# cxm12/TGSR

Measured on AMD Instinct MI355X. Metric: SR images/sec (32->256, batch 16 per GPU, one step in flight), higher is better.
Workload: dtype f32

## Files before the change

### include/tgsr_hip.h

```cpp
#ifndef TGSR_HIP_H
#define TGSR_HIP_H

#include <stdint.h>

#ifdef __cplusplus
extern "C" {
#endif

#define TGSR_OK 0
#define TGSR_EINVAL (-1)
#define TGSR_EUNSUPPORTED (-2)
#define TGSR_ELAUNCH (-3)

#define TGSR_EPI_AFFINE 0
#define TGSR_EPI_AFFINE_GLU 1

#define TGSR_ACT_NONE 0
#define TGSR_ACT_TANH_AXPY 1
#define TGSR_ACT_IDENT_AXPY 2

#define TGSR_ABI_VERSION 2
int tgsr_abi_version(void);
const char* tgsr_last_error(void);

int64_t tgsr_packed_weight_elems(int Cout, int Cin, int K);
int tgsr_pack_conv_weight(const float* w, float* wpack, int Cout, int Cin, int K, void* stream);
int tgsr_pack_conv_weight_dgrad(const float* w, float* wpack, int Cout, int Cin, int K, void* stream);

int tgsr_bn_fold(const float* weight, const float* bias, const float* running_mean, const float* running_var,
                 float eps, float* scale, float* shift, int C, void* stream);

int tgsr_conv3x3_fwd(const float* x, int64_t x_bstride, int B, int Cin, int H, int W, const float* wpack, int Cout,
                     const float* scale, const float* shift, const float* residual, int64_t res_bstride, float* out,
                     int64_t out_bstride, int epilogue, int upsample, void* stream);
int tgsr_conv3x3_fwd_plan(int B, int H, int W, int Cout, int epilogue, int upsample, int* nob, int* rows_per_wave, int* groups);

int64_t tgsr_packed_upconv_weight_elems(int Cout, int Cin);
int tgsr_pack_upconv_weight(const float* w, float* wpack, int Cout, int Cin, void* stream);
int tgsr_upconv3x3_glu_fwd(const float* x, int64_t x_bstride, int B, int Cin, int H, int W, const float* wpack, int Cout,
                           const float* scale, const float* shift, float* out, int64_t out_bstride, void* stream);

int64_t tgsr_packed_upwino_weight_elems(int Cout, int Cin);
int tgsr_pack_upwino_weight(const float* w, float* upack, int Cout, int Cin, int glu, void* stream);
int tgsr_upwino_glu_fwd(const float* x, int64_t x_bstride, int B, int Cin, int H, int W, const float* upack, int Cout,
                        const float* scale, const float* shift, float* out, int64_t out_bstride, void* stream);
int tgsr_upwino_fwd(const float* x, int64_t x_bstride, int B, int Cin, int H, int W, const float* upack, int Cout,
                    const float* scale, const float* shift, float* out, int64_t out_bstride, void* stream);

int64_t tgsr_packed_upwino4_weight_elems(int Cout, int Cin);
int tgsr_pack_upwino4_weight(const float* w, float* upack, int Cout, int Cin, int glu, void* stream);
int tgsr_upwino4_fwd(const float* x, int64_t x_bstride, int B, int Cin, int H, int W, const float* upack, int Cout,
                     const float* scale, const float* shift, float* out, int64_t out_bstride, int glu, void* stream);

int64_t tgsr_packed_wino_weight_elems(int Cout, int Cin);
int tgsr_pack_wino_weight(const float* w, float* upack, int Cout, int Cin, int glu, void* stream);
int tgsr_pack_wino_weight_dgrad(const float* w, float* upack, int Cout, int Cin, void* stream);
int tgsr_wino_conv3x3_fwd(const float* x, int64_t x_bstride, int B, int Cin, int H, int W, const float* upack, int Cout,
                          const float* scale, const float* shift, const float* residual, int64_t res_bstride,
                          float* out, int64_t out_bstride, int epilogue, void* stream);

int64_t tgsr_packed_wino4_weight_elems(int Cout, int Cin);
int tgsr_pack_wino4_weight(const float* w, float* upack, int Cout, int Cin, int glu, void* stream);
int tgsr_pack_wino4_weight_dgrad(const float* w, float* upack, int Cout, int Cin, void* stream);
int tgsr_wino4_conv3x3_fwd(const float* x, int64_t x_bstride, int B, int Cin, int H, int W, const float* upack, int Cout,
                           const float* scale, const float* shift, const float* residual, int64_t res_bstride,
                           float* out, int64_t out_bstride, int epilogue, void* stream);

int tgsr_pack_wino4_wide_weight(const float* w, float* upack, int Cout, int Cin, int glu, void* stream);
int tgsr_pack_wino4_wide_weight_dgrad(const float* w, float* upack, int Cout, int Cin, void* stream);
int tgsr_wino4_wide_stats_nslots(int B, int H, int W, int Cout);
int tgsr_wino4_wide_conv3x3_stats_fwd(const float* x, int64_t x_bstride, int B, int Cin, int H, int W, const float* upack,
                                      int Cout, float* out, int64_t out_bstride, float* stat_partial, void* stream);
int tgsr_wino4_wide_conv3x3_fwd(const float* x, int64_t x_bstride, int B, int Cin, int H, int W, const float* upack, int Cout,
                                const float* scale, const float* shift, const float* residual, int64_t res_bstride,
                                float* out, int64_t out_bstride, int epilogue, void* stream);

#define TGSR_CONV_FORM_DIRECT 0
#define TGSR_CONV_FORM_UPCONV 1
#define TGSR_CONV_FORM_UPWINO 2
#define TGSR_CONV_FORM_UPWINO4 3
#define TGSR_CONV_FORM_WINO 4
#define TGSR_CONV_FORM_WINO4 5
#define TGSR_CONV_FORM_WINO4W 6
#define TGSR_CONV_FORMS 7
#define TGSR_CONV_PLAN_FIELDS 15
int tgsr_conv3x3_form_plan(int form, const float* x, int64_t x_bstride, int B, int Cin, int H, int W, const float* pack, int Cout,
                           const float* scale, const float* shift, const float* residual, int64_t res_bstride, const float* out,
                           int64_t out_bstride, int epilogue, int upsample, int stats, int* plan);

int tgsr_conv_to3_set_pipe(int on);

int tgsr_conv_to3_fwd(const float* x, int64_t x_bstride, int B, int Cin, int H, int W, const float* w, int K,
                      int act, const float* addend, float alpha, float* out, void* stream);
#define TGSR_TO3_FORM_MFMA 0
#define TGSR_TO3_FORM_PIPE 1
#define TGSR_TO3_FORM_VEC4 2
#define TGSR_TO3_FORM_SCALAR 3
int tgsr_conv_to3_plan(const float* x, int64_t x_bstride, int B, int Cin, int H, int W, int K, const float* addend,
                       const float* out, int* form, int* tile_rows);

int tgsr_conv_to3_finish_fwd(const float* x, int64_t x_bstride, int B, int Cin, int H, int W, const float* w, int K, float* out,
                             int n, float* const* fine, const float* const* t, const float* const* s, const int64_t* numel,
                             float alpha, void* stream);

int tgsr_word_attention_fwd(const float* h, int64_t h_bstride, const float* words, const float* w_ctx,
                            const uint8_t* mask, int mask_mode, int B, int idf, int cdf, int T, int Q, float* src_ws,
                            float* c_code, int64_t c_bstride, float* attn, void* stream);

int tgsr_word_project_fwd(const float* words, const float* const* w_ctx, int nsets, int B, int idf, int cdf, int T,
                          float* src_out, void* stream);

int tgsr_bilstm_fwd(const int64_t* captions, int width, const int32_t* cap_lens, int B, int Tmax, const float* emb,
                    int ntoken, int ninput, const float* w_ih, const float* w_hh, const float* b_ih,
                    const float* b_hh, int H, float* gates_ws, float* words_emb, float* sent_emb, void* stream);

int tgsr_lstm_gate_table(const float* emb, int ntoken, int ninput, const float* w_ih, const float* b_ih,
                         const float* b_hh, int H, float* table, void* stream);
int tgsr_bilstm_table_fwd(const int64_t* captions, int width, const int32_t* cap_lens, int B, int Tmax,
                          const float* table, int ntoken, const float* w_hh, int H, float* words_emb, float* sent_emb,
                          void* stream);

#define TGSR_LSTM_RECURRENT2_128 1
#define TGSR_LSTM_RECURRENT_128 2
#define TGSR_LSTM_RECURRENT_64 3
#define TGSR_LSTM_RECURRENT_32 4
#define TGSR_LSTM_RECURRENT_GENERIC 5
int tgsr_lstm_recurrent_plan(int H, int Tmax);

// ... 327 lines not shown
```

### tgsr_amd/_lib.py

```python
import ctypes
import os
import subprocess

_HERE = os.path.dirname(os.path.abspath(__file__))
LIB_PATH = os.environ.get("TGSR_LIB_PATH") or os.path.join(_HERE, "lib", "libtgsr_hip.so")
ABI_VERSION = 2

OK, EINVAL, EUNSUPPORTED, ELAUNCH = 0, -1, -2, -3
EPI_AFFINE, EPI_AFFINE_GLU = 0, 1
ACT_NONE, ACT_TANH_AXPY, ACT_IDENT_AXPY = 0, 1, 2
TO3_FORM_MFMA, TO3_FORM_PIPE, TO3_FORM_VEC4, TO3_FORM_SCALAR = 0, 1, 2, 3
DT_BF16, DT_F16 = 1, 2
WGRAD_DIRECT, WGRAD_WINO, WGRAD_UPWINO = 0, 1, 2
WGRAD_FAMILIES = ("conv3x3_wgrad_kernel<%d,%d,%s>", "wino_wgrad_kernel<%d,%d>", "wino_wgrad_dma_kernel<%d>", "upwino_wgrad_kernel<%d>")
WGRAD_PLAN_FIELDS, WGRAD_PLAN_WS = 10, 9
TO3_BWD_PLAN_FIELDS, TO3_BWD_PLAN_WS = 4, 3
CONV_FORMS = ("direct", "upconv", "upwino", "upwino4", "wino", "wino4", "wino4w")
CONV_FAMILIES = ("conv3x3_mfma_kernel<%d,%s,%s,%d,4>", "upconv_glu_mfma_kernel", "upwino_kernel<%s>", "upwino4_kernel<%s>",
                 "wino_conv3x3_kernel<%s,%d,%s>", "wino4_conv3x3_kernel<%s,%s>", "wino4w_conv3x3_kernel<%s,%d,%s>")
CONV_PLAN_FIELDS = 15
(CONV_PLAN_FAMILY, CONV_PLAN_T, CONV_PLAN_GRID_X, CONV_PLAN_GRID_Y, CONV_PLAN_BLOCK, CONV_PLAN_TILES_X, CONV_PLAN_TILES_Y,
 CONV_PLAN_TILE_H, CONV_PLAN_TILE_W, CONV_PLAN_STAGES, CONV_PLAN_GROUPS, CONV_PLAN_NSLOTS) = (0, 1, 5, 6, 7, 8, 9, 10, 11, 12, 13, 14)

LSTM_RECURRENT = {1: "lstm_recurrent2_kernel<128,24,4>", 2: "lstm_recurrent_kernel<128>", 3: "lstm_recurrent_kernel<64>",
                  4: "lstm_recurrent_kernel<32>", 5: "lstm_recurrent_generic_kernel"}
LSTM_RECURRENT_GENERIC = 5

_vp, _i, _i64, _f, _d = ctypes.c_void_p, ctypes.c_int, ctypes.c_int64, ctypes.c_float, ctypes.c_double

SIGNATURES = {
    "tgsr_abi_version": (_i, []),
    "tgsr_last_error": (ctypes.c_char_p, []),
    "tgsr_packed_weight_elems": (_i64, [_i, _i, _i]),
    "tgsr_pack_conv_weight": (_i, [_vp, _vp, _i, _i, _i, _vp]),
    "tgsr_pack_conv_weight_dgrad": (_i, [_vp, _vp, _i, _i, _i, _vp]),
    "tgsr_bn_fold": (_i, [_vp, _vp, _vp, _vp, _f, _vp, _vp, _i, _vp]),
    "tgsr_conv3x3_fwd": (_i, [_vp, _i64, _i, _i, _i, _i, _vp, _i, _vp, _vp, _vp, _i64, _vp, _i64, _i, _i, _vp]),
    "tgsr_conv3x3_fwd_plan": (_i, [_i, _i, _i, _i, _i, _i, _vp, _vp, _vp]),
    "tgsr_packed_upconv_weight_elems": (_i64, [_i, _i]),
    "tgsr_pack_upconv_weight": (_i, [_vp, _vp, _i, _i, _vp]),
    "tgsr_upconv3x3_glu_fwd": (_i, [_vp, _i64, _i, _i, _i, _i, _vp, _i, _vp, _vp, _vp, _i64, _vp]),
    "tgsr_packed_upwino_weight_elems": (_i64, [_i, _i]),
    "tgsr_pack_upwino_weight": (_i, [_vp, _vp, _i, _i, _i, _vp]),
    "tgsr_upwino_glu_fwd": (_i, [_vp, _i64, _i, _i, _i, _i, _vp, _i, _vp, _vp, _vp, _i64, _vp]),
    "tgsr_upwino_fwd": (_i, [_vp, _i64, _i, _i, _i, _i, _vp, _i, _vp, _vp, _vp, _i64, _vp]),
    "tgsr_packed_upwino4_weight_elems": (_i64, [_i, _i]),
    "tgsr_pack_upwino4_weight": (_i, [_vp, _vp, _i, _i, _i, _vp]),
    "tgsr_upwino4_fwd": (_i, [_vp, _i64, _i, _i, _i, _i, _vp, _i, _vp, _vp, _vp, _i64, _i, _vp]),
    "tgsr_packed_wino_weight_elems": (_i64, [_i, _i]),
    "tgsr_pack_wino_weight": (_i, [_vp, _vp, _i, _i, _i, _vp]),
    "tgsr_pack_wino_weight_dgrad": (_i, [_vp, _vp, _i, _i, _vp]),
    "tgsr_wino_conv3x3_fwd": (_i, [_vp, _i64, _i, _i, _i, _i, _vp, _i, _vp, _vp, _vp, _i64, _vp, _i64, _i, _vp]),
    "tgsr_packed_wino4_weight_elems": (_i64, [_i, _i]),
    "tgsr_pack_wino4_weight": (_i, [_vp, _vp, _i, _i, _i, _vp]),
    "tgsr_pack_wino4_weight_dgrad": (_i, [_vp, _vp, _i, _i, _vp]),
    "tgsr_pack_wino4_wide_weight": (_i, [_vp, _vp, _i, _i, _i, _vp]),
    "tgsr_pack_wino4_wide_weight_dgrad": (_i, [_vp, _vp, _i, _i, _vp]),
    "tgsr_wino4_wide_stats_nslots": (_i, [_i, _i, _i, _i]),
    "tgsr_wino4_wide_conv3x3_stats_fwd": (_i, [_vp, _i64, _i, _i, _i, _i, _vp, _i, _vp, _i64, _vp, _vp]),
    "tgsr_wino4_wide_conv3x3_fwd": (_i, [_vp, _i64, _i, _i, _i, _i, _vp, _i, _vp, _vp, _vp, _i64, _vp, _i64, _i, _vp]),
    "tgsr_wino4_conv3x3_fwd": (_i, [_vp, _i64, _i, _i, _i, _i, _vp, _i, _vp, _vp, _vp, _i64, _vp, _i64, _i, _vp]),
    "tgsr_conv3x3_form_plan": (_i, [_i, _vp, _i64, _i, _i, _i, _i, _vp, _i, _vp, _vp, _vp, _i64, _vp, _i64, _i, _i, _i, _vp]),
    "tgsr_conv_to3_fwd": (_i, [_vp, _i64, _i, _i, _i, _i, _vp, _i, _i, _vp, _f, _vp, _vp]),
    "tgsr_conv_to3_plan": (_i, [_vp, _i64, _i, _i, _i, _i, _i, _vp, _vp, _vp, _vp]),
    "tgsr_word_attention_fwd": (_i, [_vp, _i64, _vp, _vp, _vp, _i, _i, _i, _i, _i, _i, _vp, _vp, _i64, _vp, _vp]),
    "tgsr_word_project_fwd": (_i, [_vp, _vp, _i, _i, _i, _i, _i, _vp, _vp]),
    "tgsr_bilstm_fwd": (_i, [_vp, _i, _vp, _i, _i, _vp, _i, _i, _vp, _vp, _vp, _vp, _i, _vp, _vp, _vp, _vp]),
    "tgsr_lstm_gate_table": (_i, [_vp, _i, _i, _vp, _vp, _vp, _i, _vp, _vp]),
    "tgsr_bilstm_table_fwd": (_i, [_vp, _i, _vp, _i, _i, _vp, _i, _vp, _i, _vp, _vp, _vp]),
    "tgsr_lstm_recurrent_plan": (_i, [_i, _i]),
    "tgsr_bilstm_train_fwd": (_i, [_vp, _vp, _i, _i, _i, _vp, _vp, _vp, _vp, _i, _vp, _vp, _vp, _vp, _vp]),
    "tgsr_bilstm_bwd": (_i, [_vp, _i, _i, _i, _vp, _vp, _vp, _vp, _vp, _vp, _vp, _vp, _vp]),
    "tgsr_damsm_words_fwd": (_i, [_vp, _vp, _vp, _i, _i, _i, _i, _f, _f, _vp, _vp, _vp]),
    "tgsr_damsm_words_bwd_ws_elems": (_i64, [_i, _i, _i]),
    "tgsr_damsm_words_bwd": (_i, [_vp, _vp, _vp, _vp, _i, _i, _i, _i, _f, _f, _vp, _vp, _vp, _vp]),
    "tgsr_func_attention_fwd": (_i, [_vp, _vp, _i, _i, _i, _i, _f, _vp, _vp, _vp]),
    "tgsr_damsm_gallery_fwd": (_i, [_vp, _vp, _vp, _vp, _i, _i, _i, _i, _i, _i, _f, _f, _vp, _vp]),
    "tgsr_sent_gallery_fwd": (_i, [_vp, _vp, _vp, _i, _i, _i, _i, _f, _f, _vp, _vp]),
    "tgsr_retrieval_ranks": (_i, [_vp, _vp, _i, _i, _vp, _vp]),
    "tgsr_feat_moments_add": (_i, [_vp, _i, _i, _i64, _vp, _vp, _vp]),
    "tgsr_poly_mmd_ws_elems": (_i64, [_i, _i]),
    "tgsr_poly_mmd_sums": (_i, [_vp, _i, _i64, _vp, _i, _i64, _vp, _vp, _i, _i, _i, _vp, _vp, _vp]),
    "tgsr_conv1x1_fwd": (_i, [_vp, _i, _i, _i, _vp, _vp, _i, _vp, _vp]),
    "tgsr_linear_fwd": (_i, [_vp, _i, _i, _vp, _vp, _i, _vp, _vp]),
    "tgsr_rowdot_fwd": (_i, [_vp, _vp, _vp, _vp, _i, _i, _vp]),
    "tgsr_ca_net_fwd": (_i, [_vp, _vp, _vp, _vp, _i, _i, _i, _vp, _vp, _vp, _vp]),
    "tgsr_rowdot_bwd": (_i, [_vp, _vp, _vp, _vp, _vp, _i, _i, _vp]),
    "tgsr_bn_train_nsplit": (_i, [_i, _i, _i]),
    "tgsr_bn_train_fwd": (_i, [_vp, _i, _i, _i, _vp, _vp, _f, _f, _vp, _vp, _i, _vp, _i64, _vp, _vp, _vp, _vp, _vp, _vp,
                               _i64, _vp, _vp]),
    "tgsr_bn_train_bwd": (_i, [_vp, _vp, _i, _i, _i, _vp, _vp, _vp, _vp, _i, _vp, _vp, _vp, _vp, _vp, _vp]),
    "tgsr_dconv_set_split": (_i, [_i]),
    "tgsr_bn_set_fuse_small": (_i, [_i]),
    "tgsr_conv_to3_set_pipe": (_i, [_i]),
    "tgsr_conv_to3_finish_fwd": (_i, [_vp, _i64, _i, _i, _i, _i, _vp, _i, _vp, _i, _vp, _vp, _vp, _vp, _f, _vp]),
    "tgsr_conv4x4s2_split_form": (_i, [_i, _i, _i, _i, _i, _i]),
    "tgsr_conv3x3_gemm_split_form": (_i, [_i, _i, _i, _i, _i, _i]),
    "tgsr_conv4x4s2_ws_elems": (_i64, [_i, _i, _i, _i, _i, _i]),
    "tgsr_conv4x4s2_fwd": (_i, [_vp, _i, _i, _i, _i, _vp, _i, _i, _vp, _vp, _vp]),
    "tgsr_conv4x4s2_dgrad": (_i, [_vp, _i, _i, _i, _i, _vp, _i, _vp, _vp, _vp]),
    "tgsr_conv4x4s2_wgrad": (_i, [_vp, _vp, _i, _i, _i, _i, _i, _vp, _vp, _vp]),
    "tgsr_conv3x3_gemm_ws_elems": (_i64, [_i, _i, _i, _i, _i, _i]),
    "tgsr_conv3x3_gemm_fwd": (_i, [_vp, _i, _i, _i, _i, _vp, _i, _vp, _vp, _vp]),
    "tgsr_conv3x3_gemm_dgrad": (_i, [_vp, _i, _i, _i, _i, _vp, _i, _vp, _vp, _vp]),
    "tgsr_conv3x3_gemm_wgrad": (_i, [_vp, _vp, _i, _i, _i, _i, _i, _vp, _vp, _vp]),
    "tgsr_leaky_relu": (_i, [_vp, _vp, _vp, _i64, _vp]),
    "tgsr_glu": (_i, [_vp, _vp, _vp, _i64, _i64, _vp]),
    "tgsr_wino_stats_nslots": (_i, [_i, _i, _i, _i]),
    "tgsr_wino_conv3x3_stats_fwd": (_i, [_vp, _i64, _i, _i, _i, _i, _vp, _i, _vp, _i64, _vp, _vp]),
    "tgsr_wino4_stats_nslots": (_i, [_i, _i, _i, _i]),
    "tgsr_wino4_conv3x3_stats_fwd": (_i, [_vp, _i64, _i, _i, _i, _i, _vp, _i, _vp, _i64, _vp, _vp]),
    "tgsr_bn_train_fwd_from_stats": (_i, [_vp, _i, _i, _i, _vp, _vp, _f, _f, _vp, _vp, _i, _vp, _i64, _vp, _i, _vp, _vp, _vp, _vp,
                                          _vp, _i64, _vp, _vp]),
# ... 150 lines not shown
```

### tgsr_amd/csrc/tgsr_winograd4.hip

```cpp
#include "tgsr_common.h"
#include "tgsr_conv_plan.h"

#include <type_traits>

namespace tgsr {

typedef __attribute__((address_space(3))) void* lds_ptr4_t;
__device__ __attribute__((aligned(16))) float g_wino4_zero[4] = {0.f, 0.f, 0.f, 0.f};

#ifdef TGSR_WINO4_STAMPS
__device__ unsigned long long g_w4stamps[8 * 8192];
#define TGSR_W4STAMP(k)                                                                                 \
  do {                                                                                                  \
    const int bid_ = blockIdx.x;                                                                        \
    if (threadIdx.x == 0 && bid_ < 8192) {                                                              \
      g_w4stamps[bid_ * 8 + (k)] = __builtin_amdgcn_s_memtime();                                        \
      if ((k) == 0) g_w4stamps[bid_ * 8 + 6] = __builtin_amdgcn_s_memrealtime();                        \
      if ((k) == 3) g_w4stamps[bid_ * 8 + 7] = __builtin_amdgcn_s_memrealtime();                        \
    }                                                                                                   \
  } while (0)
#else
#define TGSR_W4STAMP(k)
#endif

struct Wino4Args {
  const float* x;
  int64_t xbs;
  int B, Cin, H, W;
  const float* upack;
  int Cout;
  const float* scale;
  const float* shift;
  const float* res;
  int64_t rbs;
  float* out;
  int64_t obs;
  int tiles_x, tiles_y, nstages, ngroups;
  float* stat;
  int nslots;
};

constexpr int k4CK = 4;
constexpr int k4TC = 72;
constexpr int k4TR = 10;
constexpr int k4PLANE = 768;
constexpr int k4RAW = k4CK * k4PLANE;
constexpr int k4U = 9 * k4CK * 64 * 4;
constexpr int k4V = 9 * k4CK * 16 * 4;
constexpr int k4SMEM = 2 * k4U + 2 * k4RAW + 4 * k4V + 128;

__host__ __device__ constexpr int w4_row(int q, int e) {
  return (q / 3 == 0) ? ((4 * (q % 3) + e) / 6 ? 5 : 0) : ((q / 3 == 1) ? ((4 * (q % 3) + e) / 6 ? 2 : 1) : ((4 * (q % 3) + e) / 6 ? 4 : 3));
}
__host__ __device__ constexpr int w4_col(int q, int e) { return (4 * (q % 3) + e) % 6; }
__host__ __device__ constexpr int w4_pos(int i, int j) {
  return (3 * ((i == 0 || i == 5) ? 0 : ((i == 1 || i == 2) ? 1 : 2)) + (((i == 5 || i == 2 || i == 4) ? 6 : 0) + j) / 4) * 4 +
         (((i == 5 || i == 2 || i == 4) ? 6 : 0) + j) % 4;
}

typedef float f32x4w4 __attribute__((ext_vector_type(4)));

constexpr double k4P = 0.625, k4R = 1.5;
constexpr float k4P2 = (float)(k4P * k4P), k4R2 = (float)(k4R * k4R), k4PR2 = (float)(k4P * k4P * k4R * k4R),
                k4S2 = (float)(k4P * k4P + k4R * k4R), k4Pf = (float)k4P, k4Rf = (float)k4R,
                k4P3 = (float)(k4P * k4P * k4P), k4R3 = (float)(k4R * k4R * k4R);
static_assert((double)k4PR2 == k4P * k4P * k4R * k4R && (double)k4S2 == k4P * k4P + k4R * k4R && (double)k4P3 == k4P * k4P * k4P &&
              (double)k4R3 == k4R * k4R * k4R, "the interpolation points must give transform constants that are exact in fp32");
__host__ __device__ inline void w4_G(double (&G)[6][3]) {
  const double pt[4] = {k4P, -k4P, k4R, -k4R};
  G[0][0] = 1.0 / (k4P * k4P * k4R * k4R); G[0][1] = 0.0; G[0][2] = 0.0;
  for (int j = 0; j < 4; ++j) {
    double n = pt[j];
    for (int k = 0; k < 4; ++k)
      if (k != j) n *= pt[j] - pt[k];
    G[1 + j][0] = 1.0 / n; G[1 + j][1] = pt[j] / n; G[1 + j][2] = pt[j] * pt[j] / n;
  }
  G[5][0] = 0.0; G[5][1] = 0.0; G[5][2] = 1.0;
}

template <int R>
__device__ __forceinline__ void w4_bt_pair(float d0, float d1, float d2, float d3, float d4, float d5, float& oa, float& ob) {
  if (R == 0) {
    oa = fmaf(k4PR2, d0, fmaf(-k4S2, d2, d4));
    ob = fmaf(k4PR2, d1, fmaf(-k4S2, d3, d5));
  } else if (R == 1) {
    const float p = fmaf(-k4R2, d2, d4), q = fmaf(-k4R2, d1, d3);
    oa = fmaf(k4Pf, q, p);
    ob = fmaf(-k4Pf, q, p);
  } else {
    const float p = fmaf(-k4P2, d2, d4), q = fmaf(-k4P2, d1, d3);
    oa = fmaf(k4Rf, q, p);
    ob = fmaf(-k4Rf, q, p);
// ... 244 lines not shown
          rr[i][r] = f32x4w4{0.f, 0.f, 0.f, 0.f};
          if (rb && oy + r < a.H) rr[i][r] = *reinterpret_cast<const f32x4w4*>(rb + (int64_t)c * HWo + (int64_t)(oy + r) * a.W + ox);
        }
      }
#pragma unroll
      for (int i = 0; i < 4; ++i) {
        const int m = 4 * lg + i, c = grp * 64 + cb * 16 + m;
        float yv[4][4];
        ytile(i, yv);
        const float sv = aff_s[cb * 16 + m], tv = aff_s[64 + cb * 16 + m];
#pragma unroll
        for (int r = 0; r < 4; ++r) {
          if (oy + r >= a.H) continue;
          f32x4w4 o;
#pragma unroll
          for (int k = 0; k < 4; ++k) o[k] = yv[r][k] * sv + tv + rr[i][r][k];
          *reinterpret_cast<f32x4w4*>(ob + (int64_t)c * HWo + (int64_t)(oy + r) * a.W + ox) = o;
          if (STATS) {
            ssum[i] += (o[0] + o[1]) + (o[2] + o[3]);
            ssq[i] += (o[0] * o[0] + o[1] * o[1]) + (o[2] * o[2] + o[3] * o[3]);
          }
        }
      }
    }
  }
  if (STATS) {
    const int slot = ((b * a.tiles_y + ty) * a.tiles_x + tx) * 2 + g;
#pragma unroll
    for (int i = 0; i < 4; ++i) {
      float sm = ssum[i], sq = ssq[i];
#pragma unroll
      for (int o = 8; o >= 1; o >>= 1) {
        sm += __shfl_xor(sm, o);
        sq += __shfl_xor(sq, o);
      }
      if (l15 == 0) {
        const int c = grp * 64 + cb * 16 + 4 * lg + i;
        *reinterpret_cast<float2*>(a.stat + ((int64_t)c * a.nslots + slot) * 2) = make_float2(sm, sq);
      }
    }
  }
  TGSR_W4STAMP(3);
}

constexpr int k4wTR = 6, k4wPLANE = 448, k4wRAW = k4CK * k4wPLANE;
constexpr int k4wSMEM = 2 * k4wRAW + 2 * k4V + 256;
constexpr int k4wUW = 9 * 256;

template <bool GLU, int NB, bool STATS = false>
__global__ __launch_bounds__(64 * NB, 2) void wino4w_conv3x3_kernel(Wino4Args a) {
  static_assert(!(GLU && STATS), "batch statistics are taken of the raw (plain-epilogue) convolution output");
  constexpr int NR = 16 * NB;
  __shared__ __attribute__((aligned(16))) float smem[k4wSMEM];
  const int tid = threadIdx.x, lane = tid & 63, l15 = lane & 15, lg = lane >> 4;
  const int cb = __builtin_amdgcn_readfirstlane(tid >> 6);
  int t = xcd_remap(blockIdx.x, gridDim.x);
  const int grp = t % a.ngroups;
  t /= a.ngroups;
  const int tx = t % a.tiles_x;
  t /= a.tiles_x;
  const int ty = t % a.tiles_y;
  const int b = t / a.tiles_y;
  const int y0 = ty * 4, x0 = tx * 64;
  const float* xb = a.x + (int64_t)b * a.xbs;
  const uint32_t HW = (uint32_t)a.H * (uint32_t)a.W;
  float* raws = smem;
  float* vs = smem + 2 * k4wRAW;
  float* aff_s = smem + 2 * k4wRAW + 2 * k4V;

  const int npiece = NB == 8 ? ((cb == 3 || cb == 7) ? 2 : (cb >= 4 ? 1 : 0)) : (cb == 3 ? 1 : 2);
  const int piece0 = NB == 8 ? (cb == 3 ? 0 : (cb == 7 ? 2 : cb)) : 2 * cb;
  const float* rptr[2];
  int rstep[2];
#pragma unroll
  for (int k = 0; k < 2; ++k) {
    const int e = (((npiece ? piece0 : 0) + k) * 64 + lane) * 4;
    const int c = e / k4wPLANE;
    const int rem = e - c * k4wPLANE;
    const int r = rem / k4TC, j = rem - r * k4TC;
    const int gy = y0 - 1 + r, gx = x0 - 4 + j;
    const bool ok = e < k4wRAW && rem < k4wTR * k4TC && (unsigned)gy < (unsigned)a.H && (unsigned)gx < (unsigned)a.W;
    rptr[k] = ok ? xb + (uint64_t)(uint32_t)c * HW + (uint32_t)(gy * a.W + gx) : g_wino4_zero;
    rstep[k] = ok ? (int)(k4CK * HW) : 0;
  }
  const unsigned lds0 = __builtin_amdgcn_readfirstlane((unsigned)(size_t)(lds_ptr4_t)smem);
  const unsigned lds_raw = lds0 + piece0 * 1024;
  auto issue_raw = [&](int buf) {
    if (npiece >= 1) {
      asm volatile("s_mov_b32 m0, %1\n\ts_nop 0\n\tglobal_load_lds_dwordx4 %0, off" ::"v"(rptr[0]), "s"(lds_raw + buf * (k4wRAW * 4)) : "memory");
      rptr[0] += rstep[0];
    }
    if (npiece >= 2) {
      asm volatile("s_mov_b32 m0, %1\n\ts_nop 0\n\tglobal_load_lds_dwordx4 %0, off" ::"v"(rptr[1]), "s"(lds_raw + buf * (k4wRAW * 4) + 1024) : "memory");
      rptr[1] += rstep[1];
    }
  };
  const float* ubase = a.upack + ((int64_t)grp * NB + cb) * k4wUW;
  const float* const ubase0 = ubase;
  const int64_t ustride = (int64_t)a.ngroups * NB * k4wUW;
  unsigned voff[3];
#pragma unroll
  for (int k = 0; k < 3; ++k) voff[k] = (unsigned)(lane * 16 + k * 4096);
  f32x4w4 af[9];
#define TGSR_W4W_LOAD(q)                                                                                               \
  asm volatile("global_load_dwordx4 %0, %1, %2 offset:%3" : "=&v"(af[q]) : "v"(voff[(q) / 4]), "s"(ubase), "n"(((q) % 4) * 1024) : "memory")
#define TGSR_W4W_WAIT(q) asm volatile("s_waitcnt vmcnt(8)" : "+v"(af[q])::"memory")

  const int rlane = lg * k4wPLANE + 4 * l15;
  const int vwl = (lg * 16 + l15) * 4;
// ... 29 lines not shown
    if (col >= a.Cout) col = 0;
    aff_s[tid] = a.scale ? (tid < NR ? a.scale[col] : a.shift[col]) : (tid < NR ? 1.f : 0.f);
  }

  f32x4w4 M[36];
#pragma unroll
  for (int p = 0; p < 36; ++p)
#pragma unroll
    for (int i = 0; i < 4; ++i) M[p][i] = 0.f;
  const int vlane = (lg * 16 + l15) * 4;

  auto stage = [&](auto rc, auto parc, const bool MORE, const bool MORE2) {
    constexpr int R = decltype(rc)::value, PAR = decltype(parc)::value;
    if (MORE2) issue_raw(PAR);
    ubase = MORE ? ubase + ustride : ubase0;
    float d[6][6];
    if (R < 3) t_read(rc, raws + (PAR ^ 1) * k4wRAW, d);
    const float* vb = vs + PAR * k4V + vlane;
    f32x4w4 bf[3];
    bf[0] = *reinterpret_cast<const f32x4w4*>(vb);
    bf[1] = *reinterpret_cast<const f32x4w4*>(vb + (k4CK * 16 * 4));
    __builtin_amdgcn_sched_barrier(0);
#pragma unroll
    for (int q = 0; q < 9; ++q) {
      if (q + 2 < 9) bf[(q + 2) % 3] = *reinterpret_cast<const f32x4w4*>(vb + (q + 2) * (k4CK * 16 * 4));
      TGSR_W4W_WAIT(q);
#pragma unroll
      for (int e = 0; e < 4; ++e)
        M[4 * q + e] = __builtin_amdgcn_mfma_f32_16x16x4f32(af[q][e], bf[q % 3][e], M[4 * q + e], 0, 0, 0);
      __builtin_amdgcn_sched_barrier(0);
      TGSR_W4W_LOAD(q);
      if (q == 2 && R < 3) {
        t_write(rc, d, vs + (PAR ^ 1) * k4V);
        __builtin_amdgcn_sched_barrier(0);
      }
    }
    if (MORE) asm volatile("s_waitcnt vmcnt(9) lgkmcnt(0)\n\ts_barrier" ::: "memory");
  };
  auto run = [&](auto rc) {
    constexpr int R = decltype(rc)::value;
    using P0 = std::integral_constant<int, 0>;
    using P1 = std::integral_constant<int, 1>;
    issue_raw(0);
    if (a.nstages > 1) issue_raw(1);
    TGSR_W4W_LOAD(0); TGSR_W4W_LOAD(1); TGSR_W4W_LOAD(2); TGSR_W4W_LOAD(3); TGSR_W4W_LOAD(4);
    TGSR_W4W_LOAD(5); TGSR_W4W_LOAD(6); TGSR_W4W_LOAD(7); TGSR_W4W_LOAD(8);
    asm volatile("s_waitcnt vmcnt(0) lgkmcnt(0)\n\ts_barrier" ::: "memory");
    if (R < 3) {
      float d[6][6];
      t_read(rc, raws, d);
      t_write(rc, d, vs);
    }
    asm volatile("s_waitcnt lgkmcnt(0)\n\ts_barrier" ::: "memory");
    for (int st = 0; st < a.nstages; st += 2) {
      stage(rc, P0{}, true, st + 2 < a.nstages);
      stage(rc, P1{}, st + 2 < a.nstages, st + 3 < a.nstages);
    }
  };
  if (cb == 0) run(std::integral_constant<int, 0>{});
  else if (cb == 1) run(std::integral_constant<int, 1>{});
  else if (cb == 2) run(std::integral_constant<int, 2>{});
  else run(std::integral_constant<int, 3>{});
  asm volatile("s_waitcnt vmcnt(0)" ::: "memory");
#undef TGSR_W4W_LOAD
#undef TGSR_W4W_WAIT

  auto ytile = [&](int i, float (&y)[4][4]) {
    float c[4][6];
#pragma unroll
    for (int j = 0; j < 6; ++j) {
      float col[4];
      w4_at(M[w4_pos(0, j)][i], M[w4_pos(1, j)][i], M[w4_pos(2, j)][i], M[w4_pos(3, j)][i], M[w4_pos(4, j)][i], M[w4_pos(5, j)][i], col);
#pragma unroll
      for (int r = 0; r < 4; ++r) c[r][j] = col[r];
    }
#pragma unroll
    for (int r = 0; r < 4; ++r) w4_at(c[r][0], c[r][1], c[r][2], c[r][3], c[r][4], c[r][5], y[r]);
  };
  const int oy = y0, ox = x0 + 4 * l15;
  const int64_t HWo = (int64_t)a.H * a.W;
  float* __restrict__ ob = a.out + (int64_t)b * a.obs;
  const float* __restrict__ rb = a.res ? a.res + (int64_t)b * a.rbs : nullptr;
  float ssum[4] = {0.f, 0.f, 0.f, 0.f}, ssq[4] = {0.f, 0.f, 0.f, 0.f};
  if (ox < a.W) {
    if (GLU) {
#pragma unroll
      for (int p = 0; p < 2; ++p) {
        float yv[4][4], yg[4][4];
        ytile(p, yv);
        ytile(p + 2, yg);
        const int m = 4 * lg + p;
        const float sv = aff_s[cb * 16 + m], tv = aff_s[NR + cb * 16 + m], sg = aff_s[cb * 16 + m + 2], tg = aff_s[NR + cb * 16 + m + 2];
        const int c = grp * (NR / 2) + cb * 8 + 2 * lg + p;
#pragma unroll
        for (int r = 0; r < 4; ++r) {
          if (oy + r >= a.H) continue;
          f32x4w4 o;
#pragma unroll
          for (int k = 0; k < 4; ++k)
            o[k] = (yv[r][k] * sv + tv) * __builtin_amdgcn_rcpf(1.f + __expf(-(yg[r][k] * sg + tg)));
          *reinterpret_cast<f32x4w4*>(ob + (int64_t)c * HWo + (int64_t)(oy + r) * a.W + ox) = o;
        }
      }
    } else {
      f32x4w4 rr[4][4];
#pragma unroll
      for (int i = 0; i < 4; ++i) {
        const int c = grp * NR + cb * 16 + 4 * lg + i;
#pragma unroll
        for (int r = 0; r < 4; ++r) {
          rr[i][r] = f32x4w4{0.f, 0.f, 0.f, 0.f};
          if (rb && oy + r < a.H) rr[i][r] = *reinterpret_cast<const f32x4w4*>(rb + (int64_t)c * HWo + (int64_t)(oy + r) * a.W + ox);
        }
      }
#pragma unroll
      for (int i = 0; i < 4; ++i) {
        const int m = 4 * lg + i, c = grp * NR + cb * 16 + m;
        float yv[4][4];
        ytile(i, yv);
        const float sv = aff_s[cb * 16 + m], tv = aff_s[NR + cb * 16 + m];
#pragma unroll
        for (int r = 0; r < 4; ++r) {
          if (oy + r >= a.H) continue;
          f32x4w4 o;
#pragma unroll
          for (int k = 0; k < 4; ++k) o[k] = yv[r][k] * sv + tv + rr[i][r][k];
          *reinterpret_cast<f32x4w4*>(ob + (int64_t)c * HWo + (int64_t)(oy + r) * a.W + ox) = o;
          if (STATS) {
            ssum[i] += (o[0] + o[1]) + (o[2] + o[3]);
            ssq[i] += (o[0] * o[0] + o[1] * o[1]) + (o[2] * o[2] + o[3] * o[3]);
          }
        }
      }
    }
  }
  if (STATS) {
    const int slot = (b * a.tiles_y + ty) * a.tiles_x + tx;
#pragma unroll
    for (int i = 0; i < 4; ++i) {
      float sm = ssum[i], sq = ssq[i];
#pragma unroll
      for (int o = 8; o >= 1; o >>= 1) {
        sm += __shfl_xor(sm, o);
        sq += __shfl_xor(sq, o);
      }
      if (l15 == 0) {
        const int c = grp * NR + cb * 16 + 4 * lg + i;
        *reinterpret_cast<float2*>(a.stat + ((int64_t)c * a.nslots + slot) * 2) = make_float2(sm, sq);
      }
    }
  }
}

__global__ void pack_wino4w_weight_kernel(const float* __restrict__ w, float* __restrict__ up, int Cout, int Cin, int glu, int nb,
                                          int tr, int64_t total) {
  double G[6][3];
  w4_G(G);
  const int ngrp = Cout / (16 * nb);
  for (int64_t idx = (int64_t)blockIdx.x * blockDim.x + threadIdx.x; idx < total; idx += (int64_t)gridDim.x * blockDim.x) {
    const int e = (int)(idx & 3), m = (int)((idx >> 2) & 15), ci = (int)((idx >> 6) & 3);
    int64_t t = idx >> 8;
    const int q = (int)(t % 9);
    t /= 9;
    const int cbk = (int)(t % nb);
    t /= nb;
    const int grp = (int)(t % ngrp);
    const int st = (int)(t / ngrp);
    const int i = w4_row(q, e), j = w4_col(q, e);
    const int co = glu ? ((m & 2) ? (Cout >> 1) : 0) + grp * (8 * nb) + cbk * 8 + 2 * (m >> 2) + (m & 1) : grp * (16 * nb) + cbk * 16 + m;
    const int c = st * k4CK + ci;
    double u = 0.0;
    if (c < Cin) {
      const float* gw = tr ? w + ((int64_t)c * Cout + co) * 9 : w + ((int64_t)co * Cin + c) * 9;
      for (int k = 0; k < 3; ++k)
        for (int l = 0; l < 3; ++l) u += G[i][k] * (double)(tr ? gw[8 - (k * 3 + l)] : gw[k * 3 + l]) * G[j][l];
    }
    up[idx] = (float)u;
  }
}

__global__ void pack_wino4_weight_kernel(const float* __restrict__ w, float* __restrict__ up, int Cout, int Cin, int glu, int tr,
                                         int64_t total) {
  double G[6][3];
  w4_G(G);
  const int ngrp = Cout / 64;
  for (int64_t idx = (int64_t)blockIdx.x * blockDim.x + threadIdx.x; idx < total; idx += (int64_t)gridDim.x * blockDim.x) {
    const int e = (int)(idx & 3), m = (int)((idx >> 2) & 15), cbk = (int)((idx >> 6) & 3), ci = (int)((idx >> 8) & 3);
    int64_t t = idx >> 10;
    const int q = (int)(t % 9);
    t /= 9;
    const int grp = (int)(t % ngrp);
    const int st = (int)(t / ngrp);
    const int i = w4_row(q, e), j = w4_col(q, e);
    const int co = glu ? ((m & 2) ? (Cout >> 1) : 0) + grp * 32 + cbk * 8 + 2 * (m >> 2) + (m & 1) : grp * 64 + cbk * 16 + m;
    const int c = st * k4CK + ci;
    double u = 0.0;
    if (c < Cin) {
      const float* gw = tr ? w + ((int64_t)c * Cout + co) * 9 : w + ((int64_t)co * Cin + c) * 9;
      for (int k = 0; k < 3; ++k)
        for (int l = 0; l < 3; ++l) u += G[i][k] * (double)(tr ? gw[8 - (k * 3 + l)] : gw[k * 3 + l]) * G[j][l];
    }
    up[idx] = (float)u;
  }
}

}

using namespace tgsr;

#ifdef TGSR_WINO4_STAMPS
extern "C" int tgsr_debug_read_w4stamps(unsigned long long* host, int n) {
  return hipMemcpyFromSymbol(host, HIP_SYMBOL(tgsr::g_w4stamps), sizeof(unsigned long long) * n) == hipSuccess ? 0 : -3;
}
#endif

extern "C" int64_t tgsr_packed_wino4_weight_elems(int Cout, int Cin) {
  return (int64_t)((Cin + k4CK - 1) / k4CK) * 36 * k4CK * Cout;
}

static int pack_wino4_weight(const float* w, float* upack, int Cout, int Cin, int glu, int tr, void* stream) {
  return launch_pack(pack_wino4_weight_kernel, "pack_wino4_weight_kernel", 64, 2048, tgsr_packed_wino4_weight_elems(Cout, Cin), stream, w,
                     upack, Cout, Cin, glu ? 1 : 0, tr);
}

extern "C" int tgsr_pack_wino4_weight(const float* w, float* upack, int Cout, int Cin, int glu, void* stream) {
  return pack_wino4_weight(w, upack, Cout, Cin, glu, 0, stream);
}

extern "C" int tgsr_pack_wino4_weight_dgrad(const float* w, float* upack, int Cout, int Cin, void* stream) {
  return pack_wino4_weight(w, upack, Cout, Cin, 0, 1, stream);
}

extern "C" int tgsr_wino4_stats_nslots(int B, int H, int W, int Cout) {
  return conv_tiles(TGSR_CONV_FORM_WINO4, B, H, W, Cout, TGSR_EPI_AFFINE, 0, 1).nslots;
}

static int wino4_launch(int form, const ConvCall& c, float* stat, void* stream) {
  static_assert(k4CK == kConvStage && k4TR == 8 + 2 && k4TC == 64 + 8, "the plan's stage and tile are the kernels'");
  const ConvPlan p = conv_plan(form, c);
  if (p.status != TGSR_OK) return p.status;
  const bool wide = form == TGSR_CONV_FORM_WINO4W;
  Wino4Args a;
  conv_fill(a, c, p);
  a.upack = c.pack; a.res = c.res; a.rbs = c.rbs; a.nstages = p.stages; a.ngroups = p.groups; a.stat = stat; a.nslots = p.nslots;
  hipStream_t s = as_stream(stream);
  switch ((wide ? p.t[1] * 10 : 0) + p.t[0] * 2 + p.t[wide ? 2 : 1]) {
    case 2: hipLaunchKernelGGL((wino4_conv3x3_kernel<true>), p.grid, p.block, 0, s, a); break;
    case 1: hipLaunchKernelGGL((wino4_conv3x3_kernel<false, true>), p.grid, p.block, 0, s, a); break;
    case 0: hipLaunchKernelGGL((wino4_conv3x3_kernel<false>), p.grid, p.block, 0, s, a); break;
    case 82: hipLaunchKernelGGL((wino4w_conv3x3_kernel<true, 8>), p.grid, p.block, 0, s, a); break;
    case 81: hipLaunchKernelGGL((wino4w_conv3x3_kernel<false, 8, true>), p.grid, p.block, 0, s, a); break;
    case 80: hipLaunchKernelGGL((wino4w_conv3x3_kernel<false, 8>), p.grid, p.block, 0, s, a); break;
    case 42: hipLaunchKernelGGL((wino4w_conv3x3_kernel<true, 4>), p.grid, p.block, 0, s, a); break;
    case 41: hipLaunchKernelGGL((wino4w_conv3x3_kernel<false, 4, true>), p.grid, p.block, 0, s, a); break;
    case 40: hipLaunchKernelGGL((wino4w_conv3x3_kernel<false, 4>), p.grid, p.block, 0, s, a); break;
    default: return note_error("wino4_conv3x3_kernel", "the plan names no instance", 0);
  }
  return note_launch(hipGetLastError(), wide ? "wino4w_conv3x3_kernel" : "wino4_conv3x3_kernel");
}

extern "C" int tgsr_wino4_conv3x3_fwd(const float* x, int64_t x_bstride, int B, int Cin, int H, int W, const float* upack,
                                      int Cout, const float* scale, const float* shift, const float* residual,
                                      int64_t res_bstride, float* out, int64_t out_bstride, int epilogue, void* stream) {
  return wino4_launch(TGSR_CONV_FORM_WINO4, {x, x_bstride, B, Cin, H, W, upack, Cout, scale, shift, residual, res_bstride, out, out_bstride,
                                             epilogue, 0, 0}, nullptr, stream);
}

extern "C" int tgsr_wino4_conv3x3_stats_fwd(const float* x, int64_t x_bstride, int B, int Cin, int H, int W, const float* upack,
                                            int Cout, float* out, int64_t out_bstride, float* stat_partial, void* stream) {
  if (!stat_partial) return TGSR_EINVAL;
  return wino4_launch(TGSR_CONV_FORM_WINO4, {x, x_bstride, B, Cin, H, W, upack, Cout, nullptr, nullptr, nullptr, 0, out, out_bstride,
                                             TGSR_EPI_AFFINE, 0, 1}, stat_partial, stream);
}

static int pack_wino4_wide_weight(const float* w, float* upack, int Cout, int Cin, int glu, int tr, void* stream) {
  return launch_pack(pack_wino4w_weight_kernel, "pack_wino4w_weight_kernel", 64, 2048, tgsr_packed_wino4_weight_elems(Cout, Cin), stream, w,
                     upack, Cout, Cin, glu ? 1 : 0, Cout % 128 == 0 ? 8 : 4, tr);
}

extern "C" int tgsr_pack_wino4_wide_weight(const float* w, float* upack, int Cout, int Cin, int glu, void* stream) {
  return pack_wino4_wide_weight(w, upack, Cout, Cin, glu, 0, stream);
}

extern "C" int tgsr_pack_wino4_wide_weight_dgrad(const float* w, float* upack, int Cout, int Cin, void* stream) {
  return pack_wino4_wide_weight(w, upack, Cout, Cin, 0, 1, stream);
}

extern "C" int tgsr_wino4_wide_conv3x3_fwd(const float* x, int64_t x_bstride, int B, int Cin, int H, int W, const float* upack,
                                           int Cout, const float* scale, const float* shift, const float* residual,
                                           int64_t res_bstride, float* out, int64_t out_bstride, int epilogue, void* stream) {
  return wino4_launch(TGSR_CONV_FORM_WINO4W, {x, x_bstride, B, Cin, H, W, upack, Cout, scale, shift, residual, res_bstride, out, out_bstride,
                                              epilogue, 0, 0}, nullptr, stream);
}

extern "C" int tgsr_wino4_wide_stats_nslots(int B, int H, int W, int Cout) {
  return conv_tiles(TGSR_CONV_FORM_WINO4W, B, H, W, Cout, TGSR_EPI_AFFINE, 0, 1).nslots;
}

extern "C" int tgsr_wino4_wide_conv3x3_stats_fwd(const float* x, int64_t x_bstride, int B, int Cin, int H, int W,
                                                 const float* upack, int Cout, float* out, int64_t out_bstride,
                                                 float* stat_partial, void* stream) {
  if (!stat_partial) return TGSR_EINVAL;
  return wino4_launch(TGSR_CONV_FORM_WINO4W, {x, x_bstride, B, Cin, H, W, upack, Cout, nullptr, nullptr, nullptr, 0, out, out_bstride,
                                              TGSR_EPI_AFFINE, 0, 1}, stat_partial, stream);
}
```

### tgsr_amd/ops.py

```python
import collections
import ctypes
import functools
import os
from typing import Optional, Tuple

import torch

from . import _lib
from ._lib import TgsrError, check

BN_EPS = 1e-5

profile = None


def _ev():
    e = torch.cuda.Event(enable_timing=True)
    e.record()
    return e


_raw_stream = getattr(torch._C, "_cuda_getCurrentRawStream", None)


# ... 888 lines not shown
        ws = torch.empty(need, dtype=torch.float32, device=x.device) if need else None
        gconv(False, w2, x, 0, Cin, out, 0, 1, 1, 1, 0, 0, None, False, False, ws, None)
        return out
    b = None if bias is None else _f32(bias.detach(), "bias").contiguous()
    check(_lib.lib().tgsr_conv1x1_fwd(_p(x), B, Cin, H * W, _p(w2), _p(b), w2.shape[0], _p(out), _stream()),
          "tgsr_conv1x1_fwd")
    return out


def conv1x1_wgrad(dy: torch.Tensor, x: torch.Tensor) -> Optional[torch.Tensor]:
    _need_hip(dy, x)
    B, Cout, H, W = dy.shape
    Cin, K = x.shape[1], B * H * W
    if not CONV1X1_GCONV or K % 16 != 0 or K < 1024 or Cin < 64 or tuple(x.shape) != (B, Cin, H, W):
        return None
    a = _f32(dy, "dy").permute(1, 0, 2, 3).reshape(Cout, K).contiguous()
    xt = _f32(x, "x").permute(0, 2, 3, 1).reshape(1, K, Cin, 1).contiguous()
    out = torch.empty(1, Cout, Cin, 1, dtype=torch.float32, device=dy.device)
    need = gconv_ws_elems(1, Cout, Cin, 1, K)
    ws = torch.empty(need, dtype=torch.float32, device=dy.device) if need else None
    gconv(False, a, xt, 0, K, out, 0, 1, 1, 1, 0, 0, None, False, False, ws, None)
    return out.reshape(Cout, Cin)


def linear(x: torch.Tensor, w: torch.Tensor, bias: Optional[torch.Tensor] = None) -> torch.Tensor:
    _need_hip(x, w, bias)
    x = _f32(x, "x").contiguous()
    w2 = _f32(w.detach(), "w").contiguous()
    B, K = x.shape
    if w2.shape[1] != K:
        raise TgsrError("linear: weight %s vs input %s" % (tuple(w.shape), tuple(x.shape)))
    b = None if bias is None else _f32(bias.detach(), "bias").contiguous()
    if CONV1X1_GCONV and K % 16 == 0 and K >= 256:
        xt = x.t().contiguous().view(1, K, B, 1)
        img = torch.empty(1, w2.shape[0], B, 1, dtype=torch.float32, device=x.device)
        need = gconv_ws_elems(1, w2.shape[0], B, 1, K)
        ws = torch.empty(need, dtype=torch.float32, device=x.device) if need else None
        gconv(False, w2, xt, 0, K, img, 0, 1, 1, 1, 0, 0, b, False, False, ws, None)
        return img.view(w2.shape[0], B).t().contiguous()
    out = torch.empty(B, w2.shape[0], dtype=torch.float32, device=x.device)
    check(_lib.lib().tgsr_linear_fwd(_p(x), B, K, _p(w2), _p(b), w2.shape[0], _p(out), _stream()), "tgsr_linear_fwd")
    return out


def conv_to3_set_pipe(on: bool) -> bool:
    return bool(_lib.lib().tgsr_conv_to3_set_pipe(1 if on else 0))


def conv_to3_pipe() -> bool:
    L = _lib.lib()
    was = L.tgsr_conv_to3_set_pipe(1)
    L.tgsr_conv_to3_set_pipe(was)
    return bool(was)


def bn_set_fuse_small(on: bool) -> bool:
    return bool(_lib.lib().tgsr_bn_set_fuse_small(1 if on else 0))


def bn_train_fwd(raw: torch.Tensor, gamma: torch.Tensor, beta: torch.Tensor, eps: float, momentum: float,
                 running_mean: Optional[torch.Tensor], running_var: Optional[torch.Tensor], act: int = 0,
                 residual: Optional[torch.Tensor] = None, nbt: Optional[torch.Tensor] = None,
                 out: Optional[torch.Tensor] = None, stats: Optional[torch.Tensor] = None,
                 stat_partial: Optional[torch.Tensor] = None):
    _need_hip(raw, gamma, beta, running_mean, running_var, residual, nbt, out, stats, stat_partial)
    L = _lib.lib()
    B, C, Ho, Wo = raw.shape
    HW, dev = Ho * Wo, raw.device
    raw = _f32(raw, "raw")
    if not raw.is_contiguous():
        raise TgsrError("bn_train_fwd: raw must be contiguous")
    co = C // 2 if act == 1 else C
    if out is None:
        out = torch.empty(B, co, Ho, Wo, dtype=torch.float32, device=dev)
    if stats is None:
        stats = torch.empty(4, C, dtype=torch.float32, device=dev)
    res = None if residual is None else residual.contiguous()
    if stat_partial is not None:
        if (stat_partial.dim() != 3 or stat_partial.shape[0] != C or stat_partial.shape[2] != 2 or
                stat_partial.dtype != torch.float32 or not stat_partial.is_contiguous()):
            raise TgsrError("bn_train_fwd: stat_partial %s for %d channels" % (tuple(stat_partial.shape), C))
        s0, s1, s2, s3 = _rows4(stats)
        rc = L.tgsr_bn_train_fwd_from_stats(_p(raw), B, C, HW, _p(gamma), _p(beta), float(eps),
                                            float(momentum), _p(running_mean), _p(running_var), int(act), _p(res),
                                            0 if res is None else co * HW, _p(stat_partial), stat_partial.shape[1],
                                            s0, s1, s2, s3, _p(out), co * HW, _p(nbt), _stream())
        check(rc, "tgsr_bn_train_fwd_from_stats")
        return out, stats
    ws = torch.empty(C * L.tgsr_bn_train_nsplit(B, C, HW) * 4, dtype=torch.float32, device=dev)
    s0, s1, s2, s3 = _rows4(stats)
    rc = L.tgsr_bn_train_fwd(_p(raw), B, C, HW, _p(gamma), _p(beta), float(eps), float(momentum),
                             _p(running_mean), _p(running_var), int(act), _p(res), 0 if res is None else co * HW, _p(ws),
                             s0, s1, s2, s3, _p(out), co * HW, _p(nbt), _stream())
    check(rc, "tgsr_bn_train_fwd")
    return out, stats


def bn_train_bwd(dout: torch.Tensor, raw: torch.Tensor, stats: torch.Tensor, act: int, dgamma: Optional[torch.Tensor] = None,
                 dbeta: Optional[torch.Tensor] = None, draw: Optional[torch.Tensor] = None):
    _need_hip(dout, raw, stats, dgamma, dbeta, draw)
    L = _lib.lib()
    B, C, Ho, Wo = raw.shape
    HW, dev = Ho * Wo, raw.device
    dout = _f32(dout, "dout").contiguous()
    co = C // 2 if act == 1 else C
    if draw is None:
# ... 1293 lines not shown
```

Baseline: 12600.

## Make wide Winograd F(4,3) conv kernel persistent with CU-sized grid

The wide Winograd conv kernel now loops over tiles with a grid-stride loop. The launch caps the grid at one or two workgroups per compute unit, depending on the NB instance, instead of launching one workgroup per tile. This is meant to cut workgroup launch and tail overhead and to let waves stay resident. The cost is an extra barrier between tiles, a lane id recomputed each iteration, and possible load imbalance when the tile count does not divide evenly. The cap can be overridden through an environment variable or a new setter.

```diff
diff --git a/include/tgsr_hip.h b/include/tgsr_hip.h
--- a/include/tgsr_hip.h
+++ b/include/tgsr_hip.h
@@ -74,6 +74,7 @@
 int tgsr_wino4_wide_conv3x3_fwd(const float* x, int64_t x_bstride, int B, int Cin, int H, int W, const float* upack, int Cout,
                                 const float* scale, const float* shift, const float* residual, int64_t res_bstride,
                                 float* out, int64_t out_bstride, int epilogue, void* stream);
+int tgsr_wino4w_set_persist(int cap);
 
 #define TGSR_CONV_FORM_DIRECT 0
 #define TGSR_CONV_FORM_UPCONV 1
diff --git a/tgsr_amd/_lib.py b/tgsr_amd/_lib.py
--- a/tgsr_amd/_lib.py
+++ b/tgsr_amd/_lib.py
@@ -59,6 +59,7 @@
     "tgsr_wino4_wide_stats_nslots": (_i, [_i, _i, _i, _i]),
     "tgsr_wino4_wide_conv3x3_stats_fwd": (_i, [_vp, _i64, _i, _i, _i, _i, _vp, _i, _vp, _i64, _vp, _vp]),
     "tgsr_wino4_wide_conv3x3_fwd": (_i, [_vp, _i64, _i, _i, _i, _i, _vp, _i, _vp, _vp, _vp, _i64, _vp, _i64, _i, _vp]),
+    "tgsr_wino4w_set_persist": (_i, [_i]),
     "tgsr_wino4_conv3x3_fwd": (_i, [_vp, _i64, _i, _i, _i, _i, _vp, _i, _vp, _vp, _vp, _i64, _vp, _i64, _i, _vp]),
     "tgsr_conv3x3_form_plan": (_i, [_i, _vp, _i64, _i, _i, _i, _i, _vp, _i, _vp, _vp, _vp, _i64, _vp, _i64, _i, _i, _i, _vp]),
     "tgsr_conv_to3_fwd": (_i, [_vp, _i64, _i, _i, _i, _i, _vp, _i, _i, _vp, _f, _vp, _vp]),
diff --git a/tgsr_amd/csrc/tgsr_winograd4.hip b/tgsr_amd/csrc/tgsr_winograd4.hip
--- a/tgsr_amd/csrc/tgsr_winograd4.hip
+++ b/tgsr_amd/csrc/tgsr_winograd4.hip
@@ -1,6 +1,7 @@
 #include "tgsr_common.h"
 #include "tgsr_conv_plan.h"
 
+#include <atomic>
 #include <type_traits>
 
 namespace tgsr {
@@ -38,6 +39,7 @@
   int tiles_x, tiles_y, nstages, ngroups;
   float* stat;
   int nslots;
+  int ntiles;
 };
 
 constexpr int k4CK = 4;
@@ -388,9 +390,15 @@
   static_assert(!(GLU && STATS), "batch statistics are taken of the raw (plain-epilogue) convolution output");
   constexpr int NR = 16 * NB;
   __shared__ __attribute__((aligned(16))) float smem[k4wSMEM];
-  const int tid = threadIdx.x, lane = tid & 63, l15 = lane & 15, lg = lane >> 4;
-  const int cb = __builtin_amdgcn_readfirstlane(tid >> 6);
-  int t = xcd_remap(blockIdx.x, gridDim.x);
+  const int cb = __builtin_amdgcn_readfirstlane(threadIdx.x >> 6);
+  TGSR_W4STAMP(0);
+  for (unsigned w = blockIdx.x; w < (unsigned)a.ntiles; w += gridDim.x) {
+  if (w != blockIdx.x) asm volatile("s_waitcnt lgkmcnt(0)\n\ts_barrier" ::: "memory");
+  unsigned lane_z = 0;
+  asm volatile("" : "+v"(lane_z));
+  const int lane = (int)__builtin_amdgcn_mbcnt_hi(~0u, __builtin_amdgcn_mbcnt_lo(~0u, lane_z));
+  const int tid = cb * 64 + lane, l15 = lane & 15, lg = lane >> 4;
+  int t = xcd_remap((int)w, a.ntiles);
   const int grp = t % a.ngroups;
   t /= a.ngroups;
   const int tx = t % a.tiles_x;
@@ -526,6 +534,7 @@
       t_write(rc, d, vs);
     }
     asm volatile("s_waitcnt lgkmcnt(0)\n\ts_barrier" ::: "memory");
+    TGSR_W4STAMP(1);
     for (int st = 0; st < a.nstages; st += 2) {
       stage(rc, P0{}, true, st + 2 < a.nstages);
       stage(rc, P1{}, st + 2 < a.nstages, st + 3 < a.nstages);
@@ -536,8 +545,7 @@
   else if (cb == 2) run(std::integral_constant<int, 2>{});
   else run(std::integral_constant<int, 3>{});
   asm volatile("s_waitcnt vmcnt(0)" ::: "memory");
-#undef TGSR_W4W_LOAD
-#undef TGSR_W4W_WAIT
+  TGSR_W4STAMP(2);
 
   auto ytile = [&](int i, float (&y)[4][4]) {
     float c[4][6];
@@ -624,6 +632,10 @@
       }
     }
   }
+  }
+  TGSR_W4STAMP(3);
+#undef TGSR_W4W_LOAD
+#undef TGSR_W4W_WAIT
 }
 
 __global__ void pack_wino4w_weight_kernel(const float* __restrict__ w, float* __restrict__ up, int Cout, int Cin, int glu, int nb,
@@ -709,6 +721,29 @@
   return conv_tiles(TGSR_CONV_FORM_WINO4, B, H, W, Cout, TGSR_EPI_AFFINE, 0, 1).nslots;
 }
 
+static std::atomic<int> g_w4w_persist{[] {
+  const char* e = getenv("TGSR_WINO4W_PERSIST");
+  const int v = e ? atoi(e) : -1;
+  return v < -1 ? -1 : v;
+}()};
+
+extern "C" int tgsr_wino4w_set_persist(int cap) { return g_w4w_persist.exchange(cap < -1 ? -1 : cap); }
+
+static int wino4w_walkers(int nb) {
+  const int cap = g_w4w_persist.load(std::memory_order_relaxed);
+  if (cap >= 0) return cap;
+  constexpr int kMaxDev = 64;
+  static std::atomic<int> cus[kMaxDev];
+  int dev = 0;
+  if (hipGetDevice(&dev) != hipSuccess || dev < 0 || dev >= kMaxDev) return -1;
+  int n = cus[dev].load(std::memory_order_relaxed);
+  if (n == 0) {
+    if (hipDeviceGetAttribute(&n, hipDeviceAttributeMultiprocessorCount, dev) != hipSuccess || n < 1) return -1;
+    cus[dev].store(n, std::memory_order_relaxed);
+  }
+  return n * (nb == 8 ? 1 : 2);
+}
+
 static int wino4_launch(int form, const ConvCall& c, float* stat, void* stream) {
   static_assert(k4CK == kConvStage && k4TR == 8 + 2 && k4TC == 64 + 8, "the plan's stage and tile are the kernels'");
   const ConvPlan p = conv_plan(form, c);
@@ -718,16 +753,23 @@
   conv_fill(a, c, p);
   a.upack = c.pack; a.res = c.res; a.rbs = c.rbs; a.nstages = p.stages; a.ngroups = p.groups; a.stat = stat; a.nslots = p.nslots;
   hipStream_t s = as_stream(stream);
+  a.ntiles = (int)p.grid.x;
+  dim3 wg = p.grid;
+  if (wide) {
+    const int n = wino4w_walkers(p.t[1]);
+    if (n < 0) return note_error("wino4w_conv3x3_kernel", "the device does not say how many compute units it has", n);
+    if (n > 0 && (unsigned)n < wg.x) wg.x = (unsigned)n;
+  }
   switch ((wide ? p.t[1] * 10 : 0) + p.t[0] * 2 + p.t[wide ? 2 : 1]) {
     case 2: hipLaunchKernelGGL((wino4_conv3x3_kernel<true>), p.grid, p.block, 0, s, a); break;
     case 1: hipLaunchKernelGGL((wino4_conv3x3_kernel<false, true>), p.grid, p.block, 0, s, a); break;
     case 0: hipLaunchKernelGGL((wino4_conv3x3_kernel<false>), p.grid, p.block, 0, s, a); break;
-    case 82: hipLaunchKernelGGL((wino4w_conv3x3_kernel<true, 8>), p.grid, p.block, 0, s, a); break;
-    case 81: hipLaunchKernelGGL((wino4w_conv3x3_kernel<false, 8, true>), p.grid, p.block, 0, s, a); break;
-    case 80: hipLaunchKernelGGL((wino4w_conv3x3_kernel<false, 8>), p.grid, p.block, 0, s, a); break;
-    case 42: hipLaunchKernelGGL((wino4w_conv3x3_kernel<true, 4>), p.grid, p.block, 0, s, a); break;
-    case 41: hipLaunchKernelGGL((wino4w_conv3x3_kernel<false, 4, true>), p.grid, p.block, 0, s, a); break;
-    case 40: hipLaunchKernelGGL((wino4w_conv3x3_kernel<false, 4>), p.grid, p.block, 0, s, a); break;
+    case 82: hipLaunchKernelGGL((wino4w_conv3x3_kernel<true, 8>), wg, p.block, 0, s, a); break;
+    case 81: hipLaunchKernelGGL((wino4w_conv3x3_kernel<false, 8, true>), wg, p.block, 0, s, a); break;
+    case 80: hipLaunchKernelGGL((wino4w_conv3x3_kernel<false, 8>), wg, p.block, 0, s, a); break;
+    case 42: hipLaunchKernelGGL((wino4w_conv3x3_kernel<true, 4>), wg, p.block, 0, s, a); break;
+    case 41: hipLaunchKernelGGL((wino4w_conv3x3_kernel<false, 4, true>), wg, p.block, 0, s, a); break;
+    case 40: hipLaunchKernelGGL((wino4w_conv3x3_kernel<false, 4>), wg, p.block, 0, s, a); break;
     default: return note_error("wino4_conv3x3_kernel", "the plan names no instance", 0);
   }
   return note_launch(hipGetLastError(), wide ? "wino4w_conv3x3_kernel" : "wino4_conv3x3_kernel");
diff --git a/tgsr_amd/ops.py b/tgsr_amd/ops.py
--- a/tgsr_amd/ops.py
+++ b/tgsr_amd/ops.py
@@ -964,6 +964,10 @@
     was = L.tgsr_conv_to3_set_pipe(1)
     L.tgsr_conv_to3_set_pipe(was)
     return bool(was)
+
+
+def wino4w_set_persist(cap: int) -> int:
+    return int(_lib.lib().tgsr_wino4w_set_persist(int(cap)))
 
 
 def bn_set_fuse_small(on: bool) -> bool:
```

New measurement: 12860 (median of 6 runs). 1.02x the previous value.
